# raguilar011095/planet_heightmap_generation

Measured on AMD Instinct MI355X. Metric: Mcells·iter/s, terrain-post erosion stack, higher is better.
Workload: dtype f64

## Files before the change

planet_heightmap_generation_amd/csrc/basin.hip:

```cpp
#include <hip/hip_runtime.h>

#include <string>

#include "device.h"

namespace wo {

namespace {

constexpr int32_t WO_RANGE_NONE = 0x7f7f7f7f;
#ifndef WO_BASIN_RANGE_SLOTS
#define WO_BASIN_RANGE_SLOTS 256
#endif
constexpr int WO_BASIN_RANGE = WO_BASIN_RANGE_SLOTS;
constexpr int WO_BASIN_KEY_BITS = 16;
constexpr int WO_BASIN_CHASE_CAP = 1 << 16;

__device__ inline int32_t basin_root(int32_t* J, int32_t s) {
    auto ld = [&](int32_t x) { return __atomic_load_n(&J[x], __ATOMIC_RELAXED); };
    int32_t j = ld(s), tort = j;
    int power = 1, lam = 0;
    for (int it = 0; it < WO_BASIN_CHASE_CAP; ++it) {
        const int32_t jj = ld(j);
        if (jj == j) return j;
        if (jj == tort) {
            int32_t m = jj, y = ld(jj);
            for (int k = 0; k < WO_BASIN_CHASE_CAP && y != jj; ++k) {
                const int32_t yy = ld(y);
                if (yy == y) return y;
                m = y < m ? y : m;
                y = yy;
            }
            __atomic_store_n(&J[m], m, __ATOMIC_RELAXED);
            return m;
// ... 72 lines not shown
    return __builtin_fma(r1, f1, r1);
}
__device__ inline double div_tail(double x, double y, double r) {
    const double q0 = x * r;
    const double e = __builtin_fma(-y, q0, x);
    return __builtin_fma(e, r, q0);
}
__device__ inline bool factor_ok(double f, float cellDistT, bool hasT2) {
    const bool fOk = f == 0.0 || (f >= 0x1p-300 && f <= 0x1p300);
    const bool dOk = !hasT2 || (cellDistT >= 0x1p-126f && cellDistT <= 0x1p100f);
    return fOk && dOk;
}
__device__ inline SolveOut solve_apply_recip(const SolveTask& T, double factor, double y1, double r1, double y2, double r2, double er, double et, double et2, int32_t tag) {
    const bool hasT = (T.flags & 4u) != 0, tOcean = (T.flags & 1u) != 0, hasT2 = (T.flags & 8u) != 0;
    const double hr = et > 0 ? et : 0;
    double hn = div_tail(er + factor * hr, y1, r1);
    hn = hn < hr ? hr : hn;
    hn = hn < 0 ? 0 : hn;
    const double eroded = er - hn;
    const double sl = div_tail(fabs(et - et2), y2, r2);
    const double slope = hasT2 ? sl : 0.0;
    const double depositFrac = 0.5 / (1 + slope * 50);
    const double deposit = eroded * depositFrac;
    float tv = (float)(et + deposit);
    tv = ((double)tv > hn) ? (float)hn : tv;
    const bool deposits = eroded > 0 && !tOcean;
    SolveOut o;
    o.self.tag = tag; o.dep.tag = tag;
    o.self.v = hasT ? (float)hn : (float)er;
    o.dep.v = hasT ? (deposits ? tv : (float)et) : 0.0f;
    return o;
}

template <int NW, bool STATS, int LAG_ = 2>
__global__ __launch_bounds__(64 * NW, (NW <= 4 ? 4 : 2)) void k_solve_flowing(Fields F, int32_t L, const int32_t* __restrict__ rangeStart, int32_t nRanges, int32_t launchTag,
                                                               int32_t* patchPending, int32_t* totalPending, const int32_t* __restrict__ big, const uint8_t* __restrict__ longFlag,
                                                               unsigned long long* stats) {
    constexpr int SC = 64 * NW;
    constexpr int LAG = LAG_, LOOKBACK = LAG + 2;
    constexpr int RCHUNKS = (LOOKBACK + LAG + 1 <= 8) ? 8 : 16;
    constexpr int RING = RCHUNKS * SC;
    static_assert(LOOKBACK + LAG + 1 <= RCHUNKS, "ring too small for the lag");
    __shared__ unsigned long long s_ring[2 * RING];
    __shared__ int32_t s_prog[NW];
    __shared__ int32_t s_level[STATS ? RING : 1];
    __shared__ int32_t s_maxLevel;
    __shared__ unsigned long long s_passes[STATS ? NW : 1], s_readyPasses[STATS ? NW : 1], s_clk[4];
    unsigned long long myPasses = 0, myReady = 0, cRead = 0, cTurn = 0, cRest = 0, cWait = 0;
    const int tid = threadIdx.x, wave = tid >> 6, lane = tid & 63;
    const long long cStart = STATS ? clock64() : 0;
    if (STATS && tid == 0) s_maxLevel = 0;
    int32_t S, E;
    if (!block_range(rangeStart, nRanges, L, big, longFlag, S, E)) return;
    const unsigned long long* G = reinterpret_cast<const unsigned long long*>(F.out);
    for (int i = tid; i < 2 * RING; i += SC) s_ring[i] = 0;
    if (tid < NW) s_prog[tid] = 0;
    __syncthreads();
    auto ring_put = [&](int32_t word, float v, int32_t tag) {
        __hip_atomic_store(&s_ring[word], (unsigned long long)__float_as_uint(v) | ((unsigned long long)(uint32_t)tag << 32), __ATOMIC_RELAXED, __HIP_MEMORY_SCOPE_WORKGROUP);
    };
    auto ring_get = [&](int32_t word) { return __hip_atomic_load(&s_ring[word], __ATOMIC_RELAXED, __HIP_MEMORY_SCOPE_WORKGROUP); };
    auto record = [&](int32_t q) { return F.task[q < L ? q : L - 1]; };
    auto far_index = [&](int32_t g, int32_t cbase) { const int32_t sq = g >> 1; return (g >= 0 && (sq < S || sq < cbase - LOOKBACK * SC)) ? g : 0; };
    SolveTask T1 = record(S + tid), T2 = record(S + SC + tid);
    unsigned long long a0 = G[far_index(T1.predSelf, S)], a1 = G[far_index(T1.predT, S)], a2 = G[far_index(T1.predT2, S)];
    SolveOut oPrev; oPrev.self.v = 0; oPrev.self.tag = 0; oPrev.dep.v = 0; oPrev.dep.tag = 0;
    bool storePrev = false;
    uint32_t fPrev = 0; int32_t rPrev = 0, tPrev = 0;
    auto store_prev = [&](int32_t slot) {
        F.out[slot] = oPrev;
        if (F.solveFinals) {
            if (fPrev & 16u) { F.e2[rPrev] = oPrev.self.v; F.me[rPrev] = oPrev.self.v; }
            if (fPrev & 32u) { F.e2[tPrev] = oPrev.dep.v; F.me[tPrev] = oPrev.dep.v; }
        }
    };
    int32_t ci = 0;
    for (int32_t base = S; base < E; base += SC, ++ci) {
        const int32_t q = base + tid;
        const bool mine = q < E;
        const long long cw0 = STATS ? clock64() : 0;
        if (ci > LAG) {
// ... 6 lines not shown
            }
            __builtin_amdgcn_fence(__ATOMIC_ACQUIRE, "workgroup");
        }
        const long long cw1 = STATS ? clock64() : 0;
        if (storePrev) store_prev(q - SC);
        const SolveTask T = T1;
        T1 = T2;
        T2 = record(base + 2 * SC + tid);
        const unsigned long long n0 = G[far_index(T1.predSelf, base + SC)], n1 = G[far_index(T1.predT, base + SC)], n2 = G[far_index(T1.predT2, base + SC)];
        double er = T.e0r, et = T.e0t, et2 = T.e0t2;
        bool blocked = false;
        const int32_t myWord = (2 * q) & (2 * RING - 1);
        int32_t r0 = -1, r1 = -1, r2 = -1, x0 = 0, x1 = 0, x2 = 0;
        if (mine) {
            auto classify = [&](int32_t g, unsigned long long far, double& v, int32_t& rw, int32_t& expect) {
                if (g < 0) return;
                const int32_t sq = g >> 1;
                if (sq >= q) { blocked = true; return; }
                if (sq >= S && sq >= base - LOOKBACK * SC) { rw = g & (2 * RING - 1); expect = sq + 1; return; }
                const int32_t tag = (int32_t)(far >> 32);
                const bool own = sq >= S;
                if (!own || tag != launchTag) { blocked = true; return; }
                v = __uint_as_float((uint32_t)far);
            };
            classify(T.predSelf, a0, er, r0, x0); classify(T.predT, a1, et, r1, x1); classify(T.predT2, a2, et2, r2, x2);
        }
        const int32_t w0 = r0 >= 0 ? r0 : myWord, w1 = r1 >= 0 ? r1 : myWord, w2 = r2 >= 0 ? r2 : myWord;
        const bool n0b = r0 >= 0, n1b = r1 >= 0, n2b = r2 >= 0;
        const float fr = (float)er, ft = (float)et, ft2 = (float)et2;
        const SolvePrepared pre = solve_prepare(T, F.solveK, F.solveM, F.solveDt);
        const double y1 = 1 + pre.factor, y2 = (double)T.cellDistT;
        const double rc1 = recip_refined(y1), rc2 = recip_refined(y2);
        const bool recipOk = !mine || factor_ok(pre.factor, T.cellDistT, (T.flags & 8u) != 0);
        bool open = mine;
        SolveOut o; o.self.v = 0; o.self.tag = 0; o.dep.v = 0; o.dep.tag = 0;
        if (mine && blocked) { ring_put(myWord, 0.0f, -(q + 1)); ring_put(myWord + 1, 0.0f, -(q + 1)); open = false; }
        const bool waveRecipOk = !__any(!recipOk);
        if (STATS) { const long long cw2 = clock64() + (long long)(__float_as_int((float)er) & 0); cRest += (unsigned long long)(cw2 - cw1); cWait += (unsigned long long)(cw1 - cw0); }
        while (__any(open)) {
            const long long c0 = STATS ? clock64() : 0;
            const unsigned long long g0 = ring_get(w0), g1 = ring_get(w1), g2 = ring_get(w2);
            const int32_t t0 = (int32_t)(g0 >> 32), t1 = (int32_t)(g1 >> 32), t2 = (int32_t)(g2 >> 32);
            const long long c1 = STATS ? (long long)(clock64() + (t0 & 0)) : 0;
            const bool ok = (!n0b | (t0 == x0)) & (!n1b | (t1 == x1)) & (!n2b | (t2 == x2));
            const bool bad = (n0b & (t0 == -x0)) | (n1b & (t1 == -x1)) | (n2b & (t2 == -x2));
            const bool ready = open & ok;
            if (STATS) { ++myPasses; if (__any(ready)) ++myReady; }
            if (__any(ready)) {
                const double ver = n0b ? (double)__uint_as_float((uint32_t)g0) : (double)fr;
                const double vet = n1b ? (double)__uint_as_float((uint32_t)g1) : (double)ft;
                const double vet2 = n2b ? (double)__uint_as_float((uint32_t)g2) : (double)ft2;
                const SolveOut oo = waveRecipOk ? solve_apply_recip(T, pre.factor, y1, rc1, y2, rc2, ver, vet, vet2, launchTag) : solve_apply_flat(T, pre, ver, vet, vet2, launchTag);
                if (ready) {
                    o = oo;
                    if (STATS && LAG_ != 3) {
                        int32_t lv = 0;
                        if (n0b) lv = max(lv, s_level[w0 >> 1]);
                        if (n1b) lv = max(lv, s_level[w1 >> 1]);
                        if (n2b) lv = max(lv, s_level[w2 >> 1]);
                        s_level[myWord >> 1] = lv + 1;
                        atomicMax(&s_maxLevel, lv + 1);
                    }
                    ring_put(myWord, oo.self.v, q + 1); ring_put(myWord + 1, oo.dep.v, q + 1);
                    open = false;
                }
            }
            const long long c2 = STATS ? clock64() : 0;
            if (STATS) { cRead += (unsigned long long)(c1 - c0); cTurn += (unsigned long long)(c2 - c1); }
            if (__any(open & bad)) {
                if (open & bad) { blocked = true; ring_put(myWord, 0.0f, -(q + 1)); ring_put(myWord + 1, 0.0f, -(q + 1)); open = false; }
            }
        }
        oPrev = o; storePrev = mine && !blocked; fPrev = T.flags; rPrev = T.pad_[0]; tPrev = T.pad_[1];
        if (mine && blocked) { atomicAdd(&patchPending[q / WO_PATCH], 1); atomicAdd(totalPending, 1); }
        a0 = n0; a1 = n1; a2 = n2;
        if (lane == 0) __hip_atomic_store(&s_prog[wave], ci + 1, __ATOMIC_RELEASE, __HIP_MEMORY_SCOPE_WORKGROUP);
    }
    if (storePrev) store_prev(S + ((E - S - 1) / SC) * SC + tid);
    if (STATS) {
        if (lane == 0) { s_passes[wave] = myPasses; s_readyPasses[wave] = myReady; }
        if (tid == 0) { s_clk[0] = cWait; s_clk[1] = cTurn; s_clk[2] = myPasses; s_clk[3] = cRest; }
        __syncthreads();
        if (tid == 0) {
            const unsigned long long c = (unsigned long long)(clock64() - cStart);
            const unsigned long long packed = (c << 24) | (unsigned long long)(s_maxLevel & 0xffffff);
            const unsigned long long old = atomicMax(&stats[0], packed);
            if (packed > old) {
                stats[1] = (unsigned long long)(E - S);
                unsigned long long mp = 0, mr = 0;
                for (int w = 0; w < NW; ++w) { mp = s_passes[w] > mp ? s_passes[w] : mp; mr = s_readyPasses[w] > mr ? s_readyPasses[w] : mr; }
                stats[2] = mp; stats[3] = mr; stats[4] = s_clk[0]; stats[5] = s_clk[1]; stats[6] = s_clk[2]; stats[7] = s_clk[3];
            }
        }
    }
}

}

void basin_alloc(wo_planet* p) {
    const int32_t N = p->N;
    hipStream_t s = cur_stream(p);
    if (!p->d_basinJ) {
        WO_HIP(hipMalloc((void**)&p->d_basinJ, (size_t)N * 4));
        WO_HIP(hipMalloc((void**)&p->d_basinSlot, (size_t)N * 4));
        WO_HIP(hipMalloc((void**)&p->d_basinKey, (size_t)N * 4));
        WO_HIP(hipMalloc((void**)&p->d_basinVals[0], (size_t)N * 4)); WO_HIP(hipMalloc((void**)&p->d_basinVals[1], (size_t)N * 4));
        WO_HIP(hipMalloc((void**)&p->d_basinRange, ((size_t)N / 64 + 8 + WO_LONG_MAX) * 4));
        WO_HIP(hipMalloc((void**)&p->d_basinLong, (size_t)N / 64 + 8));
        WO_HIP(hipMemsetAsync(p->d_basinSlot, 0xff, (size_t)N * 4, s));
    }
}

void basin_layout(wo_planet* p, bool slotIdentity) {
    const int32_t L = p->L;
    basin_alloc(p);
    int bitsL = 1;
    while (((int64_t)1 << bitsL) < (int64_t)L) ++bitsL;
    const int shift = bitsL > WO_BASIN_KEY_BITS ? bitsL - WO_BASIN_KEY_BITS : 0;
    const int grid = blocks_for(L, 1 << 16);
    launch(p, FAM_BASIN, k_basin_jump, grid, WO_BLOCK, slotIdentity ? (const int32_t*)nullptr : (const int32_t*)p->d_patchOrder, p->d_basinJ, L, (int32_t)shift, p->d_basinKey);
    const int rangeT = WO_BASIN_RANGE;
    const int nRanges = (int)(((int64_t)L + rangeT - 1) / rangeT);
    launch(p, FAM_BASIN, k_basin_keys, grid, WO_BLOCK, (const int32_t*)p->d_land[p->landCur], (const uint32_t*)p->d_basinKey, L, p->d_keys[0], p->d_basinVals[0],
           (int32_t)(p->opt.basinScramble ? 1 : 0), p->d_basinRange, (int32_t)(nRanges + 1));
    uint32_t* const kb[2] = {p->d_keys[0], p->d_keys[1]};
    int32_t* const vb[2] = {p->d_basinVals[0], p->d_basinVals[1]};
    const int sorted = radix_sort_pairs(p, FAM_BASIN_SORT, kb, vb, L, 0, 16 , p->d_basinSlot, radix_scratch(p, 1), p->N, p->rsFlip[1]);
    launch(p, FAM_BASIN, k_basin_slots, blocks_for(L, 4096), WO_BLOCK, (const int32_t*)p->d_basinVals[sorted], (const uint32_t*)p->d_keys[sorted], (int32_t*)nullptr, L, p->d_basinRange, (int32_t)rangeT);
    launch(p, FAM_BASIN, k_basin_long, blocks_for(nRanges), WO_BLOCK, (const int32_t*)p->d_basinRange, (int32_t)nRanges, L, p->d_basinRange + nRanges + 1, p->d_basinLong);
}

void basin_solve_launch(wo_planet* p, const Fields& F, int32_t launchTag, int32_t* totalPending) {
    const int nRanges = (int)(((int64_t)p->L + WO_BASIN_RANGE - 1) / WO_BASIN_RANGE);
    ++p->basinLaunches;
    const int32_t* big = (const int32_t*)(p->d_basinRange + nRanges + 1);
    const uint8_t* flag = (const uint8_t*)p->d_basinLong;
    const int grid = nRanges + WO_LONG_MAX;
    launch(p, FAM_SOLVE_BASIN, k_solve_flowing<2, false>, grid, 128, F, p->L, (const int32_t*)p->d_basinRange, (int32_t)nRanges, launchTag, p->d_patchPending, totalPending, big, flag, (unsigned long long*)nullptr);
}

void basin_free(wo_planet* p) {
    if (p->d_basinJ) (void)hipFree(p->d_basinJ);
    if (p->d_basinSlot) (void)hipFree(p->d_basinSlot);
    if (p->d_basinKey) (void)hipFree(p->d_basinKey);
    for (auto& v : p->d_basinVals) { if (v) (void)hipFree(v); v = nullptr; }
    if (p->d_basinRange) (void)hipFree(p->d_basinRange);
    if (p->d_basinLong) (void)hipFree(p->d_basinLong);
    p->d_basinLong = nullptr;
    p->d_basinJ = nullptr; p->d_basinSlot = nullptr; p->d_basinKey = nullptr; p->d_basinRange = nullptr;
}

}
```

planet_heightmap_generation_amd/csrc/device.h:

```cpp
#pragma once
#include <hip/hip_runtime.h>

#include <cstdint>
#include <cstdio>
#include <map>
#include <string>
#include <vector>

#include "host_util.h"

#include "erode_ops.h"
#include "flood_ops.h"
#include "wo_internal.h"

namespace wo {

struct HipError { std::string msg; };

#define WO_HIP(call)                                                                                   \
    do {                                                                                               \
        hipError_t e_ = (call);                                                                        \
        if (e_ != hipSuccess)                                                                          \
            throw ::wo::HipError{std::string(#call) + " -> " + hipGetErrorString(e_) + " (" + __FILE__ + ":" + \
                                 std::to_string(__LINE__) + ")"};                                      \
// ... 29 lines not shown
extern const char* const kFamilyNames[FAM_COUNT];

}

struct wo_ctx {
    int device = 0;
    hipStream_t stream = nullptr;
    hipDeviceProp_t prop{};
};

struct wo_flood_gpu {
    int64_t version = -1; int32_t L = 0, cap = 0, nSeeds = 0;
    int32_t *off = nullptr, *adj = nullptr, *cell = nullptr, *seedIdx = nullptr, *seeds = nullptr; double* nz = nullptr;
    float* e = nullptr;
    wo::FlHead *A = nullptr, *P = nullptr, *F = nullptr;
    unsigned long long *Astk = nullptr, *Pstk = nullptr, *Fstk = nullptr;
    int32_t *fdEpoch = nullptr, *inDirty = nullptr; uint8_t* isPending = nullptr;
    int32_t* lists[5] = {nullptr, nullptr, nullptr, nullptr, nullptr};
    void* ctrl = nullptr; void* h_ctrl = nullptr;
    int32_t *jump = nullptr, *outPar = nullptr, *outRoot = nullptr; float* outSurf = nullptr;
    int32_t *h_par = nullptr, *h_root = nullptr; float* h_surf = nullptr;
};

namespace wo {
struct Options {
    bool layoutIndex = false;
    bool tileLds = false;
    bool floodDevice = false;
    bool floodTiming = false;
    bool stageTimingAll = false;
    int  relaxedSortEvery = 1;
    bool relaxedFull = false;
    bool basinScramble = false;
    long long carveBudgetMs = 200;
    int  carveBlocks = 0;
    static Options from_env();
};
}

struct wo_planet {
    wo_ctx* ctx = nullptr;
    wo::Options opt;
    int32_t N = 0, E = 0, maxDeg = 0;
    wo::hvec<int32_t> h_off, h_adj;
    wo::hvec<float> h_xyz;
    wo::hvec<uint8_t> h_ocean;
    bool h_ocean_valid = false;
    float* h_pinned = nullptr;
    int32_t* h_count = nullptr;
    float* d_redoE = nullptr; int32_t* d_pendingEver = nullptr; int64_t redoCalls = 0;
    unsigned long long *h_word = nullptr, *d_word = nullptr; uint32_t wordSerial = 0;
    wo::FloodScratch flood;
    wo::FloodExchange floodX;
    void* floodLink = nullptr; void (*floodLinkFree)(void*) = nullptr;
    wo_flood_gpu fgpu;

    int32_t *d_off = nullptr, *d_adj = nullptr;
    float *d_dist = nullptr, *d_xyz = nullptr;
    float *d_e = nullptr, *d_e2 = nullptr, *d_hot = nullptr, *d_orig = nullptr;
    uint8_t *d_ocean = nullptr, *d_coast = nullptr;
    int64_t mirrorMaskVersion = -1;
    uint8_t* d_oceanKnown = nullptr; int32_t* d_maskDiff = nullptr; bool oceanKnownValid = false;
    bool hot_valid = false;
    float* d_savedE = nullptr; uint8_t* d_savedOcean = nullptr; bool saved = false;
    uint8_t* d_tables = nullptr;
    bool scratch = false;
    bool landIdentity = false;
    int64_t floodPrefixMirror = -1, floodPrefixStatic = -1;
    bool floodPrefixOk = false;
    int32_t *d_landIdx = nullptr, *d_land[2] = {nullptr, nullptr}, *d_rank = nullptr;
    int32_t* d_landInit = nullptr; int64_t oceanVersion = 0, landListsOcean = -1; bool landListsMirror = false; int32_t landListsL = -1;
    uint32_t* d_keys[2] = {nullptr, nullptr};
    float *d_cellDist = nullptr, *d_flow = nullptr;
    wo::SolveTask* d_task = nullptr; wo::SolveOut* d_out = nullptr; int32_t *d_haloSend = nullptr, *d_haloRecv = nullptr; float *d_haloBuf = nullptr, *h_haloBuf = nullptr; int32_t nHaloSend = 0, nHaloRecv = 0;
    int32_t* d_flowCnt = nullptr; wo::TargetRank* d_tr = nullptr; wo::EventList* d_ev = nullptr; float* d_me = nullptr;
    int32_t *d_carveSlot = nullptr, *d_carveDeps = nullptr, *d_carveDepCnt = nullptr, *d_carveDepPos = nullptr; uint32_t* d_rs[2] = {nullptr, nullptr}; int rsFlip[2] = {0, 0};    wo::CarveRec* d_carveRecs = nullptr; wo::CarveExpect* d_carveExpect = nullptr; unsigned long long* d_carveG = nullptr;    int32_t* d_carveSlotDone = nullptr; int64_t carveCap = 0;
    unsigned long long* d_accCnt = nullptr;
    int32_t *d_ftLr = nullptr, *d_ftParent = nullptr, *d_ftExtCnt = nullptr; uint32_t* d_ftInflow = nullptr; unsigned long long* d_ftRootAcc = nullptr;
    int32_t *d_jump = nullptr, *d_nj = nullptr;
    int32_t* d_doneAt = nullptr;
    double* d_totalExcess = nullptr;
    float *d_glac = nullptr, *d_iceFlow = nullptr;
    int32_t *d_iceTarget = nullptr, *d_arank = nullptr;
    uint8_t* d_iceUp = nullptr;
    int32_t *d_patchOrder = nullptr, *d_slotOf = nullptr, *d_patchPending = nullptr, *d_patchTotals = nullptr, *d_patchBlk = nullptr; int64_t patchVersion = -1; bool patchMirror = false; int32_t numPatches = 0; int64_t lastPatchLaunches = 1; int64_t solveCalls = 0;
    hipStream_t side = nullptr; hipEvent_t evFork = nullptr, evJoin = nullptr; bool onSide = false;
    uint32_t* d_basinKey = nullptr; int32_t* d_basinVals[2] = {nullptr, nullptr}; int32_t *d_basinJ = nullptr, *d_basinSlot = nullptr, *d_basinRange = nullptr; uint8_t* d_basinLong = nullptr; int64_t basinLaunches = 0; wo::Affine* d_affine[2] = {nullptr, nullptr};    int64_t solvePassSerial = 0;
    int32_t* h_patchTotals = nullptr;
    int32_t *d_listA = nullptr, *d_listB = nullptr, *d_counters = nullptr;
    void* d_sortTemp = nullptr; size_t sortTempBytes = 0;
    int landCur = 0;
    int32_t L = 0;

    struct Import {
        uint8_t* img = nullptr; int64_t imgCap = 0;
        int32_t* label = nullptr;
        uint8_t* flags = nullptr;
        int32_t* lists = nullptr;
        uint8_t* seedOcean = nullptr;
        int32_t* blockCounts = nullptr;
        int32_t* totals = nullptr; int32_t* h_totals = nullptr;
    } imp;

    struct wo_wind_block* wind = nullptr;

    struct Mirror {
        bool built = false, active = false;
        int32_t *perm = nullptr, *inv = nullptr, *off = nullptr, *adj = nullptr;
        float *dist = nullptr, *xyz = nullptr, *e = nullptr, *e2 = nullptr, *hot = nullptr;
        uint8_t *ocean = nullptr, *coast = nullptr;
        wo::hvec<int32_t> h_perm, h_morton;
        wo::hvec<uint8_t> h_mask;
        int64_t version = 0;
        int32_t *o_off = nullptr, *o_adj = nullptr; float *o_dist = nullptr, *o_xyz = nullptr, *o_e = nullptr, *o_e2 = nullptr;
        uint8_t *o_ocean = nullptr, *o_coast = nullptr;
    } mirror;

    hipEvent_t evStart = nullptr, evStop = nullptr;
    bool profiling = false;
// ... 67 lines not shown
```

planet_heightmap_generation_amd/csrc/erode_ops.h:

```cpp
#pragma once
#include <cmath>
#include <cstdint>
#include <cstring>

#include "noise.h"

namespace wo {

constexpr int WO_MAX_DEG = 24;
constexpr int32_t WO_NOT_DONE = 0x7fffffff;

#ifndef WO_TASK_ALIGN
#define WO_TASK_ALIGN 16
#endif
struct alignas(WO_TASK_ALIGN) SolveTask {
    int32_t predSelf, predT, predT2;
    uint32_t flags;
    float e0r, e0t, e0t2;
    float cellDistT;
    double factor;
    int32_t pad_[2];
};
static_assert(sizeof(SolveTask) == 48, "one 48-byte record per task");
#ifndef WO_PATCH_CELLS
// ... 503 lines not shown
    const double eroded = er - hn;
    float tval = (float)et;
    if (eroded > 0 && !(T.flags & 1u)) {
        double slope = 0;
        if (T.flags & 8u) slope = fabs(et - et2) / S.cellDistT;
        const double depositFrac = 0.5 / (1 + slope * 50);
        const double deposit = eroded * depositFrac;
        tval = (float)(et + deposit);
        if ((double)tval > hn) tval = (float)hn;
    }
    o.self.v = (float)hn; o.dep.v = tval;
    return o;
}
WO_HD inline SolveOut solve_apply_flat(const SolveTask& T, const SolvePrepared& S, double er, double et, double et2, int32_t tag) {
    const bool hasT = (T.flags & 4u) != 0, tOcean = (T.flags & 1u) != 0, hasT2 = (T.flags & 8u) != 0;
    const double hr = et > 0 ? et : 0;
    double hn = (er + S.factor * hr) / S.onePlusFactor;
    hn = hn < hr ? hr : hn;
    hn = hn < 0 ? 0 : hn;
    const double eroded = er - hn;
    const double sl = fabs(et - et2) / S.cellDistT;
    const double slope = hasT2 ? sl : 0.0;
    const double depositFrac = 0.5 / (1 + slope * 50);
    const double deposit = eroded * depositFrac;
    float tv = (float)(et + deposit);
    tv = ((double)tv > hn) ? (float)hn : tv;
    const bool deposits = eroded > 0 && !tOcean;
    SolveOut o;
    o.self.tag = tag; o.dep.tag = tag;
    o.self.v = hasT ? (float)hn : (float)er;
    o.dep.v = hasT ? (deposits ? tv : (float)et) : 0.0f;
    return o;
}
WO_HD inline SolveOut solve_compute(const SolveTask& T, double er, double et, double et2, int32_t tag, double K, double m, double dt) {
    return solve_apply(T, solve_prepare(T, K, m, dt), er, et, et2, tag);
}

WO_HD inline bool solve_task(const Fields& F, int32_t r, int32_t round, double K, double m, double dt) {
    const SolveTask T = F.task[r];
    const Granule* G = reinterpret_cast<const Granule*>(F.out);
    double er = T.e0r, et = T.e0t, et2 = T.e0t2;
    if (T.predSelf >= 0) { const Granule g = G[T.predSelf]; if (g.tag == 0 || !(g.tag < round)) return false; er = g.v; }
    if (T.predT >= 0)    { const Granule g = G[T.predT];    if (g.tag == 0 || !(g.tag < round)) return false; et = g.v; }
    if (T.predT2 >= 0)   { const Granule g = G[T.predT2];   if (g.tag == 0 || !(g.tag < round)) return false; et2 = g.v; }
    F.out[r] = solve_compute(T, er, et, et2, round, K, m, dt);
    return true;
}

WO_HD inline int32_t latest_event_cell(const Fields& F, int32_t x) {
    int32_t best = -1, bestRank = 0x7fffffff;
    { const TargetRank v = F.tr[x]; if (v.target >= 0) { best = x; bestRank = v.rank; } }
    int32_t b, nbs[WO_ROW];
    const int deg = load_row(F, x, b, nbs);
    if (deg <= WO_ROW) {
        TargetRank q[WO_ROW];
#pragma unroll
        for (int k = 0; k < WO_ROW; ++k) q[k] = F.tr[nbs[k]];
#pragma unroll
        for (int k = 0; k < WO_ROW; ++k) if (k < deg && q[k].target == x && q[k].rank < bestRank) { best = nbs[k]; bestRank = q[k].rank; }
    } else {
        for (int32_t j = b; j < b + deg; ++j) {
            const int32_t n = F.adj[j];
            const TargetRank v = F.tr[n];
            if (v.target != x) continue;
            if (v.rank < bestRank) { best = n; bestRank = v.rank; }
        }
// ... 453 lines not shown
```

planet_heightmap_generation_amd/csrc/planet.hip:

```cpp
#include <hip/hip_runtime.h>

#include <algorithm>
#include <atomic>
#include <chrono>
#include <cmath>
#include <cstring>

#include "../../include/worogen.h"
#include "device.h"
#include "elevation_host.h"
#include "elevation_kernels.h"
#include "kernels_impl.h"
#include "flood_kernels.h"
#include "elevation_bfs.h"
#include "noise.h"

namespace wo {

const char* const kFamilyNames[FAM_COUNT] = {
    "coast_flags", "smooth_elevation", "sharpen_ridges", "soil_creep", "warp_terrain", "noise_eval", "synthetic_terrain",
    "ocean_from_elevation", "sort_keys", "sort_radix", "rank_scatter", "receivers", "flow_climb",
    "flow_final", "solve_setup", "solve_round", "solve_final", "thermal_excess", "thermal_apply",
    "glac_index", "ice_receivers", "ice_round", "carve_setup", "carve_round", "moraine_fjord", "glacial_blend", "solve_patch", "elev_collisions", "elev_uplift_fused", "plate_grid", "plate_project", "smooth_field", "flood_eval", "flood_apply", "flood_misc", "climate_sweeps", "basin_layout", "basin_sort", "solve_basin", "flow_tiles", "misc", "event_pair_empty", "event_pair_noop_kernel", "event_pair_two_noop_kernels"};

// ... 458 lines not shown
        const int32_t N = p->N;
        launch(p, FAM_MISC, k_mirror_gather_f32, blocks_for(N, 4096), WO_BLOCK, (const float*)p->d_e, (const int32_t*)M.perm, M.e, N);
        launch(p, FAM_MISC, k_mirror_gather_u8, blocks_for(N, 4096), WO_BLOCK, (const uint8_t*)p->d_ocean, (const int32_t*)M.perm, M.ocean, N);
        M.o_off = p->d_off; M.o_adj = p->d_adj; M.o_dist = p->d_dist; M.o_xyz = p->d_xyz; M.o_e = p->d_e; M.o_e2 = p->d_e2; M.o_ocean = p->d_ocean; M.o_coast = p->d_coast;
        point_at_mirror(M.e, M.e2);
        M.active = on = true;
    }
    void suspend() {
        if (!on) return;
        auto& M = p->mirror;
        launch(p, FAM_MISC, k_mirror_scatter_f32, blocks_for(p->N, 4096), WO_BLOCK, (const float*)p->d_e, (const int32_t*)M.perm, M.o_e, p->N);
        cur = p->d_e; cur2 = p->d_e2;
        point_at_planet();
    }
    void resume() {
        if (!on) return;
        auto& M = p->mirror;
        launch(p, FAM_MISC, k_mirror_gather_f32, blocks_for(p->N, 4096), WO_BLOCK, (const float*)M.o_e, (const int32_t*)M.perm, cur, p->N);
        point_at_mirror(cur, cur2);
    }
    void finish() {
        if (!on) return;
        suspend();
        p->mirror.active = on = false;
    }
    ~MirrorScope() { if (on) { point_at_planet(); p->mirror.active = false; } }
};

static void ensure_side_stream(wo_planet* p) {
    if (p->side) return;
    int prLeast = 0, prGreatest = 0;
    WO_HIP(hipDeviceGetStreamPriorityRange(&prLeast, &prGreatest));
    WO_HIP(hipStreamCreateWithPriority(&p->side, hipStreamNonBlocking, prGreatest));
    WO_HIP(hipEventCreateWithFlags(&p->evFork, hipEventDisableTiming)); WO_HIP(hipEventCreateWithFlags(&p->evJoin, hipEventDisableTiming));
}

struct RedoWithChecks {};

struct ErodeCall {
    wo_planet* p;
    int32_t hIters; double K, m, dt; int32_t tIters; double talus, kThermal; int32_t gIters; double gStrength; bool checkEveryPass;
    int32_t total, midIter; double gCarve, gConv, gDep, gFjord;
    int gridN, gridL = 0;
    StageClock clk; MirrorScope mir; FloodRun floodRun;
    int64_t sorts = 0, maxSolve = 0, patchLaunches = 0, basinPasses = 0, basinLeftoverPasses = 0, iceRounds = 0, carveRounds = 0, carveActive = 0, carveFlowLeft = 0;
    double floodHostMs = 0;
    ErodeCall(wo_planet* pl, int32_t h, double K_, double m_, double dt_, int32_t t, double talus_, double kT, int32_t g, double gs, bool check)
        : p(pl), hIters(h), K(K_), m(m_), dt(dt_), tIters(t), talus(talus_), kThermal(kT), gIters(std::max(g, 0)), gStrength(gs != gs ? 0 : gs),
          checkEveryPass(check), total(std::max(hIters, std::max(tIters, gIters))), midIter((int32_t)std::floor(total * 0.75 + 0.5)),
          gridN(xcd_grid(pl->N)), clk(pl), mir(pl) {
        const double gScale = gIters > 0 ? 1.0 / gIters : 0;
        gCarve = 0.02 * gScale; gConv = 0.01 * gScale; gDep = 0.005 * gScale; gFjord = 0.015 * gScale;
    }
    void stats(bool mirrored) const {
        p->erodeStats = {{"land_cells", (double)p->L}, {"mirror_layout", mirrored ? 1.0 : 0.0}, {"iterations", (double)total}, {"sorts", (double)sorts},
                         {"solve_launches_max_per_pass", (double)maxSolve}, {"solve_patch_launches_total", (double)patchLaunches},
                         {"solve_basin_passes", (double)basinPasses}, {"solve_basin_passes_with_leftovers", (double)basinLeftoverPasses},
                         {"flow_two_level", (p->d_ftLr && p->landIdentity && hIters > 0) ? 1.0 : 0.0}, {"ice_rounds_total", (double)iceRounds},
                         {"carve_rounds_total", (double)carveRounds}, {"carve_active_total", (double)carveActive}, {"carve_flow_launches_with_leftovers", (double)carveFlowLeft}, {"solve_check_every_pass", checkEveryPass ? 1.0 : 0.0}, {"calls_run_again_with_checks", (double)p->redoCalls}, {"flood_stage_ms", floodHostMs},
                         {"flood_device_pass1_ms", floodRun.deviceMs}, {"flood_device_rounds", (double)floodRun.rounds}, {"flood_device_epochs", (double)floodRun.epochs},
                         {"flood_device_evaluations", (double)floodRun.evals}, {"flood_equal_key_decisions", (double)floodRun.ties}, {"flood_pass1_on_host", (floodRun.usedDevice && !floodRun.fellBack) ? 0.0 : 1.0},
                         {"flood_host_calls", (double)floodRun.host.calls}, {"flood_host_serial_pass1", (double)floodRun.host.serialPass1}, {"flood_host_tie_groups", (double)floodRun.host.tieGroups}, {"flood_host_contested", (double)floodRun.host.contested},
                         {"flood_host_open_parents", (double)floodRun.host.openParents}, {"flood_host_unresolved", (double)floodRun.host.unresolved},
                         {"flood_host_path_redo", (double)floodRun.host.pathRedo}, {"flood_host_replays", (double)floodRun.host.replays}, {"flood_host_replayed_landmasses", (double)floodRun.host.replayedLandmasses}, {"flood_host_pass1_ms", floodRun.host.pass1Ms},
                         {"flood_host_pass23_ms", floodRun.host.pass23Ms},
                         {"relaxed_sort_every", (double)p->opt.relaxedSortEvery}, {"relaxed_full", p->opt.relaxedFull ? 1.0 : 0.0}, {"flood_exchange_calls", (double)p->floodX.calls}, {"flood_exchange_gathers", (double)p->floodX.gathers}, {"flood_exchange_whole_planet_floods", (double)p->floodX.globalFloods}, {"flood_exchange_received", (double)p->floodX.received}};
    }
// ... 194 lines not shown
    if (!basin) return;
    ensure_side_stream(p);
    if (tilesBeforeFork) {
        launch(p, FAM_FLOW_TILES, k_flow_tiles<false>, flow_tile_count(p->L), FT_THREADS, F, FT);
        launch(p, FAM_FLOW_TILES, k_flow_root_links, blocks_for(p->L, 4096), WO_BLOCK, F, FT);
    }
    WO_HIP(hipEventRecord(p->evFork, s));
    WO_HIP(hipStreamWaitEvent(p->side, p->evFork, 0));
    p->onSide = true;
    try { basin_layout(p, slotIdentity); } catch (...) { p->onSide = false; throw; }
    p->onSide = false;
    WO_HIP(hipEventRecord(p->evJoin, p->side));
}
static void erode_flow(ErodeCall& c, const Fields& F, const FlowTiles& FT, int32_t* donorCnt, bool flowTiles, bool tilesBeforeFork, bool clearOut) {
    wo_planet* p = c.p;
    c.clk.begin("flow");
    if (flowTiles) {
        const int tiles = flow_tile_count(p->L);
        if (!tilesBeforeFork) {
            launch(p, FAM_FLOW_TILES, k_flow_tiles<false>, tiles, FT_THREADS, F, FT);
            launch(p, FAM_FLOW_TILES, k_flow_root_links, blocks_for(p->L, 4096), WO_BLOCK, F, FT);
        }
        launch(p, FAM_FLOW_TILES, k_flow_root_climb, blocks_for(p->L, 4096), WO_BLOCK, F, FT);
        launch(p, FAM_FLOW_TILES, k_flow_tiles<true>, tiles, FT_THREADS, F, FT);
    } else
        launch(p, FAM_FLOW_SNAP, k_flow_climb, c.gridL, WO_BLOCK, F, (const int32_t*)p->d_flowCnt, (int32_t)0x7fffffff);
    Fields Ff = F;
    if (p->opt.relaxedFull) Ff.ev = nullptr;
    launch(p, FAM_FLOW_FINAL, k_flow_final, c.gridL, WO_BLOCK, Ff, donorCnt, clearOut ? p->d_out : (SolveOut*)nullptr);
    c.clk.end();
}
static void erode_solve_basin(ErodeCall& c, Fields F, int32_t iter) {
    wo_planet* p = c.p; hipStream_t s = p->ctx->stream;
    WO_HIP(hipStreamWaitEvent(s, p->evJoin, 0));
    F.slotOf = p->d_basinSlot; F.solveLean = 1;
    const bool unchecked = !c.checkEveryPass; F.solveFinals = unchecked ? 1 : 0;
    launch(p, FAM_SOLVE_SETUP, k_solve_setup_batched<true>, c.gridL, WO_BLOCK, F, p->d_patchPending, (int32_t)p->numPatches, p->d_patchTotals, (int32_t)WO_PATCH_TOTAL_SLOTS);
    int32_t passTag = 1;
    if (unchecked) {
        if (p->solvePassSerial >= 0x3ff00000) { WO_HIP(hipMemsetAsync(p->d_out, 0, (size_t)p->N * sizeof(SolveOut), s)); p->solvePassSerial = 0; }
        passTag = (1 << 20) + (int32_t)(++p->solvePassSerial);
    }
    const int64_t r = run_solve_patches(p, F, c.K, c.m, c.dt, unchecked, passTag);
    ++c.basinPasses; if (r > 1) ++c.basinLeftoverPasses;
    c.patchLaunches += r; c.maxSolve = std::max(c.maxSolve, r);
    if (!unchecked) launch(p, FAM_SOLVE_FINAL, k_solve_final, c.gridL, WO_BLOCK, F, p->d_e2, (iter < c.tIters) ? p->d_me : (float*)nullptr);
}
static void erode_solve_affine(ErodeCall& c, const Fields& F) {
    wo_planet* p = c.p;
    if (!p->d_affine[0]) { p->d_affine[0] = dalloc<Affine>((size_t)p->N); p->d_affine[1] = dalloc<Affine>((size_t)p->N); }
    launch(p, FAM_SOLVE_SETUP, k_affine_init, c.gridL, WO_BLOCK, F, p->d_affine[0]);
    int cur = 0;
    for (int q = 0; q < 12; ++q, cur ^= 1) launch(p, FAM_SOLVE_ROUND, k_affine_jump, c.gridL, WO_BLOCK, F, (const Affine*)p->d_affine[cur], p->d_affine[cur ^ 1]);
    launch(p, FAM_SOLVE_FINAL, k_affine_apply, c.gridL, WO_BLOCK, F, (const Affine*)p->d_affine[cur], p->d_e2);
}
static void hydraulic_step(ErodeCall& c, int32_t iter) {
    wo_planet* p = c.p;
    Fields F = p->fields();
    F.solveK = c.K; F.solveM = c.m; F.solveDt = c.dt;
    const bool basin = !p->opt.relaxedFull;
    const bool slotIdentity = c.mir.on && p->mirror.h_mask.size() == (size_t)p->N;
    if (basin) { basin_alloc(p); F.basinMslot = slotIdentity ? nullptr : p->d_slotOf; }
    const bool flowTiles = p->landIdentity;
    FlowTiles FT = flowTiles ? flow_tiles_buffers(p) : FlowTiles{};
    const bool tilesBeforeFork = basin && flowTiles && slotIdentity;
    if (tilesBeforeFork) FT.basinJ = p->d_basinJ;
    int32_t* const donorCnt = flowTiles ? (int32_t*)nullptr : p->d_flowCnt;
    erode_receivers(c, F, FT, donorCnt, basin, slotIdentity, tilesBeforeFork);
    erode_flow(c, F, FT, donorCnt, flowTiles, tilesBeforeFork, basin && c.checkEveryPass);
    c.clk.begin("solve");
    if (basin) erode_solve_basin(c, F, iter); else erode_solve_affine(c, F);
    swap_elev(p);
    c.clk.end();
}
static void thermal_step(ErodeCall& c, bool afterSolve) {
// ... 107 lines not shown
    ~DevBufs() { for (void* b : bufs) (void)hipFree(b); }
    template <class T> T* up(const T* host, size_t n, hipStream_t s) {
        if (!host) return nullptr;
        void* d = nullptr; WO_HIP(hipMalloc(&d, std::max<size_t>(n, 1) * sizeof(T))); bufs.push_back(d);
        WO_HIP(hipMemcpyAsync(d, host, n * sizeof(T), hipMemcpyHostToDevice, s));
        return (T*)d;
    }
    template <class T> T* alloc(size_t n) { void* d = nullptr; WO_HIP(hipMalloc(&d, std::max<size_t>(n, 1) * sizeof(T))); bufs.push_back(d); return (T*)d; }
};
ClimateMesh climate_mesh(const wo_planet* p) { ClimateMesh M; M.N = p->N; M.off = p->d_off; M.adj = p->d_adj; M.xyz = p->d_xyz; return M; }
}


using namespace wo;

#define WO_TRY try {
#define WO_CATCH(fn)                                                                   \
    } catch (const HipError& e) { set_error(std::string(fn) + ": " + e.msg); return 2; } \
      catch (const std::exception& e) { set_error(std::string(fn) + ": " + e.what()); return 3; }

Options Options::from_env() {
    auto str = [](const char* n) { const char* v = std::getenv(n); return std::string(v ? v : ""); };
    auto on = [](const char* n) { const char* v = std::getenv(n); return v && std::atoi(v) != 0; };
    auto set = [](const char* n) { return std::getenv(n) != nullptr; };
    Options o;
    o.layoutIndex = str("WO_LAYOUT") == "index";
    o.tileLds = on("WO_TILE_LDS");
    o.floodDevice = str("WO_FLOOD") == "device";
    o.floodTiming = set("WO_FLOOD_TIMING");
    o.stageTimingAll = str("WO_STAGE_TIMING") == "all";
    if (set("WO_RELAXED_SORT_EVERY")) o.relaxedSortEvery = std::max(1, std::atoi(std::getenv("WO_RELAXED_SORT_EVERY")));
    o.relaxedFull = str("WO_RELAXED") == "full";
    o.basinScramble = test_hook_int("basin_scramble", 0) != 0;
    o.carveBudgetMs = test_hook_int("carve_budget_ms", 200);
    o.carveBlocks = (int)std::max<long long>(0, test_hook_int("carve_blocks", 0));
    return o;
}

float* wo::smooth_field_resident(wo_planet* p, float* a, float* b, int32_t passes) {
    Fields F = p->fields();
    for (int32_t pass = 0; pass < passes; ++pass) {
        launch(p, FAM_SMOOTH_FIELD, k_smooth_field, xcd_grid(p->N), WO_BLOCK, F, (const float*)a, b);
        std::swap(a, b);
    }
    return a;
}

bool wo::check_planet(wo_planet* p, const char* fn) {
    if (!p) { set_error(std::string(fn) + ": null planet handle"); return false; }
    p->opt = Options::from_env();
    hipError_t e = hipSetDevice(p->ctx->device);
    if (e != hipSuccess) { set_error(std::string(fn) + ": hipSetDevice failed: " + hipGetErrorString(e)); return false; }
    return true;
}

static void erode_composite_checked(wo_planet* p, int32_t hIters, double K, double m, double dt, int32_t tIters, double talus,
                                    double kThermal, int32_t gIters, double gStrength) {
    if (hIters <= 0 || p->floodX.on) { erode_composite(p, hIters, K, m, dt, tIters, talus, kThermal, gIters, gStrength, true); return; }
    hipStream_t s = p->ctx->stream;
    if (!p->d_redoE) p->d_redoE = dalloc<float>((size_t)p->N);
    if (!p->d_pendingEver) p->d_pendingEver = dalloc<int32_t>(16);
    WO_HIP(hipMemcpyAsync(p->d_redoE, p->d_e, (size_t)p->N * sizeof(float), hipMemcpyDeviceToDevice, s));
    WO_HIP(hipMemsetAsync(p->d_pendingEver, 0, 16 * sizeof(int32_t), s));
    try {
        erode_composite(p, hIters, K, m, dt, tIters, talus, kThermal, gIters, gStrength, false);
    } catch (const RedoWithChecks&) {
// ... 82 lines not shown
        if (neighborDist) {
            WO_HIP(hipMemcpyAsync(p->d_dist, neighborDist, (size_t)E * 4, hipMemcpyHostToDevice, s));
        } else {
            std::vector<float> nd(E);
            neighbor_dist(N, adjOffset, adjList, r_xyz, nd.data());
            WO_HIP(hipMemcpyAsync(p->d_dist, nd.data(), (size_t)E * 4, hipMemcpyHostToDevice, s));
            WO_HIP(hipStreamSynchronize(s));
        }
        WO_HIP(hipMemsetAsync(p->d_e, 0, (size_t)N * 4, s));
        WO_HIP(hipMemsetAsync(p->d_ocean, 0, (size_t)N, s));
        WO_HIP(hipEventCreate(&p->evStart)); WO_HIP(hipEventCreate(&p->evStop));
        WO_HIP(hipStreamSynchronize(s));
        return p;
    } catch (const HipError& e) {
        set_error(std::string("wo_planet_create: ") + e.msg);
        if (p) wo_planet_destroy(p);
        return nullptr;
    }
}

void wo_planet_destroy(wo_planet* p) {
    if (!p) return;
    (void)hipSetDevice(p->ctx->device);
    (void)hipStreamSynchronize(p->ctx->stream);
    dfree(p->d_off); dfree(p->d_adj); dfree(p->d_dist); dfree(p->d_xyz); dfree(p->d_e); dfree(p->d_e2); dfree(p->d_hot); dfree(p->d_orig);
    flood_gpu_free(p->fgpu);
    if (p->floodLink && p->floodLinkFree) p->floodLinkFree(p->floodLink);
    p->floodLink = nullptr;
    basin_free(p);
    import_free(p);
    wind_free(p);
    if (p->side) { (void)hipStreamSynchronize(p->side); (void)hipStreamDestroy(p->side); p->side = nullptr; }
    if (p->evFork) { (void)hipEventDestroy(p->evFork); p->evFork = nullptr; }
    if (p->evJoin) { (void)hipEventDestroy(p->evJoin); p->evJoin = nullptr; }
    mirror_free(p);
    dfree(p->d_ocean); dfree(p->d_coast); dfree(p->d_tables); dfree(p->d_savedE); dfree(p->d_savedOcean);
    if (p->d_oceanKnown) { (void)hipFree(p->d_oceanKnown); p->d_oceanKnown = nullptr; } if (p->d_maskDiff) { (void)hipFree(p->d_maskDiff); p->d_maskDiff = nullptr; }
    dfree(p->d_landInit); dfree(p->d_landIdx); dfree(p->d_land[0]); dfree(p->d_land[1]); dfree(p->d_keys[0]); dfree(p->d_keys[1]); dfree(p->d_rank);
    dfree(p->d_cellDist); dfree(p->d_flow); dfree(p->d_task); dfree(p->d_out); dfree(p->d_flowCnt); dfree(p->d_tr); dfree(p->d_ev); dfree(p->d_me); dfree(p->d_haloSend); dfree(p->d_haloRecv); dfree(p->d_haloBuf); if (p->h_haloBuf) { (void)hipHostFree(p->h_haloBuf); p->h_haloBuf = nullptr; } dfree(p->d_carveSlot); dfree(p->d_redoE); dfree(p->d_pendingEver); for (auto& r : p->d_rs) { if (r) (void)hipFree(r); r = nullptr; } dfree(p->d_carveG); dfree(p->d_carveExpect); dfree(p->d_carveRecs); dfree(p->d_carveSlotDone); dfree(p->d_carveDeps); dfree(p->d_carveDepCnt); dfree(p->d_carveDepPos); dfree(p->d_ftLr); dfree(p->d_ftParent); dfree(p->d_affine[0]); dfree(p->d_affine[1]); dfree(p->d_ftExtCnt); dfree(p->d_ftInflow); dfree(p->d_ftRootAcc); dfree(p->d_accCnt); dfree(p->d_jump); dfree(p->d_nj);
    dfree(p->d_doneAt); dfree(p->d_totalExcess);
    dfree(p->d_glac); dfree(p->d_iceFlow); dfree(p->d_iceTarget); dfree(p->d_arank); dfree(p->d_iceUp);
    dfree(p->d_patchOrder); dfree(p->d_slotOf); dfree(p->d_patchPending); dfree(p->d_patchTotals); dfree(p->d_patchBlk);
    dfree(p->d_listA); dfree(p->d_listB); dfree(p->d_counters);
    if (p->h_patchTotals) (void)hipHostFree(p->h_patchTotals);
    if (p->d_sortTemp) (void)hipFree(p->d_sortTemp);
    if (p->h_pinned) (void)hipHostFree(p->h_pinned);
    if (p->h_count) (void)hipHostFree(p->h_count);
    if (p->h_word) { (void)hipHostFree(p->h_word); p->h_word = nullptr; }
    for (auto& pe : p->pending) { (void)hipEventDestroy(pe.a); (void)hipEventDestroy(pe.b); }
    for (auto& b : p->stageBrackets) { (void)hipEventDestroy(b.a); (void)hipEventDestroy(b.b); }
    for (auto e : p->eventPool) (void)hipEventDestroy(e);
    if (p->evStart) (void)hipEventDestroy(p->evStart);
    if (p->evStop) (void)hipEventDestroy(p->evStop);
    delete p;
}

int wo_planet_upload(wo_planet* p, const float* r_elevation, const uint8_t* r_isOcean) {
    if (!check_planet(p, "wo_planet_upload")) return 1;
    WO_TRY
    hipStream_t s = p->ctx->stream;
    if (r_elevation) WO_HIP(hipMemcpyAsync(p->d_e, r_elevation, (size_t)p->N * 4, hipMemcpyHostToDevice, s));
    if (r_isOcean) {
        WO_HIP(hipMemcpyAsync(p->d_ocean, r_isOcean, (size_t)p->N, hipMemcpyHostToDevice, s));
        if (p->h_ocean.size() != (size_t)p->N || std::memcmp(p->h_ocean.data(), r_isOcean, (size_t)p->N) != 0) {
            p->h_ocean.assign(r_isOcean, r_isOcean + p->N);
            p->flood.staticValid = false; ++p->oceanVersion;
// ... 677 lines not shown
```

Baseline: 6272.

## Split basin solve into height and deferred deposit phases; wait on slots event earlier

The flowing solve kernel now computes and publishes only the height value on the critical dependency chain. The deposit value, which needs a second division, is computed later during passes where no lane in the wave was ready, so idle spin passes absorb that work. Separately, the main stream now waits on a new event recorded right after the basin sort, and only waits for the full join before the patch solve, so setup overlaps the slot and long-range kernels. This adds an extra loop state and more branching, and the deposit write can lag behind readers that need it.

```diff
diff --git a/planet_heightmap_generation_amd/csrc/basin.hip b/planet_heightmap_generation_amd/csrc/basin.hip
--- a/planet_heightmap_generation_amd/csrc/basin.hip
+++ b/planet_heightmap_generation_amd/csrc/basin.hip
@@ -1,5 +1,7 @@
 #include <hip/hip_runtime.h>
 
+#include <cstdio>
+#include <cstdlib>
 #include <string>
 
 #include "device.h"
@@ -138,10 +140,12 @@
     return o;
 }
 
+struct SolveDivRecip { double y, r; __device__ double operator()(double x) const { return div_tail(x, y, r); } };
+
 template <int NW, bool STATS, int LAG_ = 2>
 __global__ __launch_bounds__(64 * NW, (NW <= 4 ? 4 : 2)) void k_solve_flowing(Fields F, int32_t L, const int32_t* __restrict__ rangeStart, int32_t nRanges, int32_t launchTag,
                                                                int32_t* patchPending, int32_t* totalPending, const int32_t* __restrict__ big, const uint8_t* __restrict__ longFlag,
-                                                               unsigned long long* stats) {
+                                                               int32_t depositEveryPass, unsigned long long* stats) {
     constexpr int SC = 64 * NW;
     constexpr int LAG = LAG_, LOOKBACK = LAG + 2;
     constexpr int RCHUNKS = (LOOKBACK + LAG + 1 <= 8) ? 8 : 16;
@@ -151,8 +155,8 @@
     __shared__ int32_t s_prog[NW];
     __shared__ int32_t s_level[STATS ? RING : 1];
     __shared__ int32_t s_maxLevel;
-    __shared__ unsigned long long s_passes[STATS ? NW : 1], s_readyPasses[STATS ? NW : 1], s_clk[4];
-    unsigned long long myPasses = 0, myReady = 0, cRead = 0, cTurn = 0, cRest = 0, cWait = 0;
+    __shared__ unsigned long long s_passes[STATS ? NW : 1], s_readyPasses[STATS ? NW : 1], s_depositPasses[STATS ? NW : 1], s_clk[6];
+    unsigned long long myPasses = 0, myReady = 0, myDeposit = 0, cRead = 0, cTurn = 0, cDeposit = 0, cRest = 0, cWait = 0;
     const int tid = threadIdx.x, wave = tid >> 6, lane = tid & 63;
     const long long cStart = STATS ? clock64() : 0;
     if (STATS && tid == 0) s_maxLevel = 0;
@@ -225,12 +229,15 @@
         const double y1 = 1 + pre.factor, y2 = (double)T.cellDistT;
         const double rc1 = recip_refined(y1), rc2 = recip_refined(y2);
         const bool recipOk = !mine || factor_ok(pre.factor, T.cellDistT, (T.flags & 8u) != 0);
-        bool open = mine;
+        bool open = mine, owes = false;
         SolveOut o; o.self.v = 0; o.self.tag = 0; o.dep.v = 0; o.dep.tag = 0;
         if (mine && blocked) { ring_put(myWord, 0.0f, -(q + 1)); ring_put(myWord + 1, 0.0f, -(q + 1)); open = false; }
         const bool waveRecipOk = !__any(!recipOk);
+        const SolveDivRecip byY1{y1, rc1}, byY2{y2, rc2};
+        const SolveDivBy flatY1{pre.onePlusFactor}, flatY2{pre.cellDistT};
+        double hEt = 0, hEt2 = 0, hHn = 0, hEroded = 0; bool hDeposits = false;
         if (STATS) { const long long cw2 = clock64() + (long long)(__float_as_int((float)er) & 0); cRest += (unsigned long long)(cw2 - cw1); cWait += (unsigned long long)(cw1 - cw0); }
-        while (__any(open)) {
+        while (__any(open | owes)) {
             const long long c0 = STATS ? clock64() : 0;
             const unsigned long long g0 = ring_get(w0), g1 = ring_get(w1), g2 = ring_get(w2);
             const int32_t t0 = (int32_t)(g0 >> 32), t1 = (int32_t)(g1 >> 32), t2 = (int32_t)(g2 >> 32);
@@ -238,14 +245,16 @@
             const bool ok = (!n0b | (t0 == x0)) & (!n1b | (t1 == x1)) & (!n2b | (t2 == x2));
             const bool bad = (n0b & (t0 == -x0)) | (n1b & (t1 == -x1)) | (n2b & (t2 == -x2));
             const bool ready = open & ok;
-            if (STATS) { ++myPasses; if (__any(ready)) ++myReady; }
-            if (__any(ready)) {
+            const bool anyReady = __any(ready);
+            if (STATS) { ++myPasses; if (anyReady) ++myReady; }
+            if (anyReady) {
                 const double ver = n0b ? (double)__uint_as_float((uint32_t)g0) : (double)fr;
                 const double vet = n1b ? (double)__uint_as_float((uint32_t)g1) : (double)ft;
                 const double vet2 = n2b ? (double)__uint_as_float((uint32_t)g2) : (double)ft2;
-                const SolveOut oo = waveRecipOk ? solve_apply_recip(T, pre.factor, y1, rc1, y2, rc2, ver, vet, vet2, launchTag) : solve_apply_flat(T, pre, ver, vet, vet2, launchTag);
+                const SolveHeight H = waveRecipOk ? solve_height_phase(T.flags, pre.factor, byY1, ver, vet) : solve_height_phase(T.flags, pre.factor, flatY1, ver, vet);
                 if (ready) {
-                    o = oo;
+                    o.self.v = H.selfV; o.self.tag = launchTag;
+                    hEt = vet; hEt2 = vet2; hHn = H.hn; hEroded = H.eroded; hDeposits = H.deposits;
                     if (STATS && LAG_ != 3) {
                         int32_t lv = 0;
                         if (n0b) lv = max(lv, s_level[w0 >> 1]);
@@ -254,12 +263,22 @@
                         s_level[myWord >> 1] = lv + 1;
                         atomicMax(&s_maxLevel, lv + 1);
                     }
-                    ring_put(myWord, oo.self.v, q + 1); ring_put(myWord + 1, oo.dep.v, q + 1);
-                    open = false;
+                    ring_put(myWord, H.selfV, q + 1);
+                    open = false; owes = true;
                 }
             }
             const long long c2 = STATS ? clock64() : 0;
-            if (STATS) { cRead += (unsigned long long)(c1 - c0); cTurn += (unsigned long long)(c2 - c1); }
+            if ((!anyReady | (depositEveryPass != 0)) && __any(owes)) {
+                if (STATS) ++myDeposit;
+                const float dv = waveRecipOk ? solve_deposit_phase(T.flags, byY2, hEt, hEt2, hHn, hEroded, hDeposits) : solve_deposit_phase(T.flags, flatY2, hEt, hEt2, hHn, hEroded, hDeposits);
+                if (owes) {
+                    o.dep.v = dv; o.dep.tag = launchTag;
+                    ring_put(myWord + 1, dv, q + 1);
+                    owes = false;
+                }
+            }
+            const long long c3 = STATS ? clock64() : 0;
+            if (STATS) { cRead += (unsigned long long)(c1 - c0); cTurn += (unsigned long long)(c2 - c1); cDeposit += (unsigned long long)(c3 - c2); }
             if (__any(open & bad)) {
                 if (open & bad) { blocked = true; ring_put(myWord, 0.0f, -(q + 1)); ring_put(myWord + 1, 0.0f, -(q + 1)); open = false; }
             }
@@ -271,8 +290,8 @@
     }
     if (storePrev) store_prev(S + ((E - S - 1) / SC) * SC + tid);
     if (STATS) {
-        if (lane == 0) { s_passes[wave] = myPasses; s_readyPasses[wave] = myReady; }
-        if (tid == 0) { s_clk[0] = cWait; s_clk[1] = cTurn; s_clk[2] = myPasses; s_clk[3] = cRest; }
+        if (lane == 0) { s_passes[wave] = myPasses; s_readyPasses[wave] = myReady; s_depositPasses[wave] = myDeposit; }
+        if (tid == 0) { s_clk[0] = cWait; s_clk[1] = cTurn; s_clk[2] = myPasses; s_clk[3] = cRest; s_clk[4] = cDeposit; s_clk[5] = cRead; }
         __syncthreads();
         if (tid == 0) {
             const unsigned long long c = (unsigned long long)(clock64() - cStart);
@@ -280,9 +299,10 @@
             const unsigned long long old = atomicMax(&stats[0], packed);
             if (packed > old) {
                 stats[1] = (unsigned long long)(E - S);
-                unsigned long long mp = 0, mr = 0;
-                for (int w = 0; w < NW; ++w) { mp = s_passes[w] > mp ? s_passes[w] : mp; mr = s_readyPasses[w] > mr ? s_readyPasses[w] : mr; }
+                unsigned long long mp = 0, mr = 0, md = 0;
+                for (int w = 0; w < NW; ++w) { mp = s_passes[w] > mp ? s_passes[w] : mp; mr = s_readyPasses[w] > mr ? s_readyPasses[w] : mr; md = s_depositPasses[w] > md ? s_depositPasses[w] : md; }
                 stats[2] = mp; stats[3] = mr; stats[4] = s_clk[0]; stats[5] = s_clk[1]; stats[6] = s_clk[2]; stats[7] = s_clk[3];
+                stats[8] = md; stats[9] = s_clk[4]; stats[10] = s_clk[5];
             }
         }
     }
@@ -319,6 +339,7 @@
     uint32_t* const kb[2] = {p->d_keys[0], p->d_keys[1]};
     int32_t* const vb[2] = {p->d_basinVals[0], p->d_basinVals[1]};
     const int sorted = radix_sort_pairs(p, FAM_BASIN_SORT, kb, vb, L, 0, 16 , p->d_basinSlot, radix_scratch(p, 1), p->N, p->rsFlip[1]);
+    WO_HIP(hipEventRecord(p->evSlots, cur_stream(p)));
     launch(p, FAM_BASIN, k_basin_slots, blocks_for(L, 4096), WO_BLOCK, (const int32_t*)p->d_basinVals[sorted], (const uint32_t*)p->d_keys[sorted], (int32_t*)nullptr, L, p->d_basinRange, (int32_t)rangeT);
     launch(p, FAM_BASIN, k_basin_long, blocks_for(nRanges), WO_BLOCK, (const int32_t*)p->d_basinRange, (int32_t)nRanges, L, p->d_basinRange + nRanges + 1, p->d_basinLong);
 }
@@ -329,7 +350,20 @@
     const int32_t* big = (const int32_t*)(p->d_basinRange + nRanges + 1);
     const uint8_t* flag = (const uint8_t*)p->d_basinLong;
     const int grid = nRanges + WO_LONG_MAX;
-    launch(p, FAM_SOLVE_BASIN, k_solve_flowing<2, false>, grid, 128, F, p->L, (const int32_t*)p->d_basinRange, (int32_t)nRanges, launchTag, p->d_patchPending, totalPending, big, flag, (unsigned long long*)nullptr);
+#ifdef WO_BASIN_STATS_BUILD
+    const char* at = std::getenv("WO_BASIN_STATS");
+    if (at && p->basinLaunches == std::atoll(at)) {
+        hipStream_t s = cur_stream(p);
+        unsigned long long* d = nullptr; unsigned long long h[16] = {0};
+        WO_HIP(hipMalloc((void**)&d, sizeof h)); WO_HIP(hipMemsetAsync(d, 0, sizeof h, s));
+        launch(p, FAM_SOLVE_BASIN, k_solve_flowing<2, true>, grid, 128, F, p->L, (const int32_t*)p->d_basinRange, (int32_t)nRanges, launchTag, p->d_patchPending, totalPending, big, flag, (int32_t)(p->opt.solveDepositEveryPass ? 1 : 0), d);
+        WO_HIP(hipMemcpyAsync(h, d, sizeof h, hipMemcpyDeviceToHost, s)); WO_HIP(hipStreamSynchronize(s)); (void)hipFree(d);
+        std::fprintf(stderr, "basin stats: launch %lld slowest range: clocks %llu slots %llu depth %llu | passes %llu height %llu deposit %llu | wave 0 clocks: wait %llu read %llu height %llu deposit %llu rest %llu\n",
+                     (long long)p->basinLaunches, h[0] >> 24, h[1], h[0] & 0xffffffull, h[2], h[3], h[8], h[4], h[10], h[5], h[9], h[7]);
+        return;
+    }
+#endif
+    launch(p, FAM_SOLVE_BASIN, k_solve_flowing<2, false>, grid, 128, F, p->L, (const int32_t*)p->d_basinRange, (int32_t)nRanges, launchTag, p->d_patchPending, totalPending, big, flag, (int32_t)(p->opt.solveDepositEveryPass ? 1 : 0), (unsigned long long*)nullptr);
 }
 
 void basin_free(wo_planet* p) {
diff --git a/planet_heightmap_generation_amd/csrc/device.h b/planet_heightmap_generation_amd/csrc/device.h
--- a/planet_heightmap_generation_amd/csrc/device.h
+++ b/planet_heightmap_generation_amd/csrc/device.h
@@ -85,6 +85,7 @@
     int  relaxedSortEvery = 1;
     bool relaxedFull = false;
     bool basinScramble = false;
+    bool solveDepositEveryPass = false;
     long long carveBudgetMs = 200;
     int  carveBlocks = 0;
     static Options from_env();
@@ -137,7 +138,7 @@
     int32_t *d_iceTarget = nullptr, *d_arank = nullptr;
     uint8_t* d_iceUp = nullptr;
     int32_t *d_patchOrder = nullptr, *d_slotOf = nullptr, *d_patchPending = nullptr, *d_patchTotals = nullptr, *d_patchBlk = nullptr; int64_t patchVersion = -1; bool patchMirror = false; int32_t numPatches = 0; int64_t lastPatchLaunches = 1; int64_t solveCalls = 0;
-    hipStream_t side = nullptr; hipEvent_t evFork = nullptr, evJoin = nullptr; bool onSide = false;
+    hipStream_t side = nullptr; hipEvent_t evFork = nullptr, evSlots = nullptr, evJoin = nullptr; bool onSide = false;
     uint32_t* d_basinKey = nullptr; int32_t* d_basinVals[2] = {nullptr, nullptr}; int32_t *d_basinJ = nullptr, *d_basinSlot = nullptr, *d_basinRange = nullptr; uint8_t* d_basinLong = nullptr; int64_t basinLaunches = 0; wo::Affine* d_affine[2] = {nullptr, nullptr};    int64_t solvePassSerial = 0;
     int32_t* h_patchTotals = nullptr;
     int32_t *d_listA = nullptr, *d_listB = nullptr, *d_counters = nullptr;
diff --git a/planet_heightmap_generation_amd/csrc/erode_ops.h b/planet_heightmap_generation_amd/csrc/erode_ops.h
--- a/planet_heightmap_generation_amd/csrc/erode_ops.h
+++ b/planet_heightmap_generation_amd/csrc/erode_ops.h
@@ -559,6 +559,33 @@
     o.dep.v = hasT ? (deposits ? tv : (float)et) : 0.0f;
     return o;
 }
+struct SolveDivBy { double y; WO_HD double operator()(double x) const { return x / y; } };
+struct SolveHeight { double hn, eroded; float selfV; bool deposits; };
+template <class Div>
+WO_HD inline SolveHeight solve_height_phase(uint32_t flags, double factor, const Div& byOnePlusFactor, double er, double et) {
+    const bool hasT = (flags & 4u) != 0, tOcean = (flags & 1u) != 0;
+    const double hr = et > 0 ? et : 0;
+    double hn = byOnePlusFactor(er + factor * hr);
+    hn = hn < hr ? hr : hn;
+    hn = hn < 0 ? 0 : hn;
+    SolveHeight H;
+    H.hn = hn;
+    H.eroded = er - hn;
+    H.deposits = H.eroded > 0 && !tOcean;
+    H.selfV = hasT ? (float)hn : (float)er;
+    return H;
+}
+template <class Div>
+WO_HD inline float solve_deposit_phase(uint32_t flags, const Div& byCellDistT, double et, double et2, double hn, double eroded, bool deposits) {
+    const bool hasT = (flags & 4u) != 0, hasT2 = (flags & 8u) != 0;
+    const double sl = byCellDistT(fabs(et - et2));
+    const double slope = hasT2 ? sl : 0.0;
+    const double depositFrac = 0.5 / (1 + slope * 50);
+    const double deposit = eroded * depositFrac;
+    float tv = (float)(et + deposit);
+    tv = ((double)tv > hn) ? (float)hn : tv;
+    return hasT ? (deposits ? tv : (float)et) : 0.0f;
+}
 WO_HD inline SolveOut solve_compute(const SolveTask& T, double er, double et, double et2, int32_t tag, double K, double m, double dt) {
     return solve_apply(T, solve_prepare(T, K, m, dt), er, et, et2, tag);
 }
diff --git a/planet_heightmap_generation_amd/csrc/planet.hip b/planet_heightmap_generation_amd/csrc/planet.hip
--- a/planet_heightmap_generation_amd/csrc/planet.hip
+++ b/planet_heightmap_generation_amd/csrc/planet.hip
@@ -514,7 +514,7 @@
     int prLeast = 0, prGreatest = 0;
     WO_HIP(hipDeviceGetStreamPriorityRange(&prLeast, &prGreatest));
     WO_HIP(hipStreamCreateWithPriority(&p->side, hipStreamNonBlocking, prGreatest));
-    WO_HIP(hipEventCreateWithFlags(&p->evFork, hipEventDisableTiming)); WO_HIP(hipEventCreateWithFlags(&p->evJoin, hipEventDisableTiming));
+    WO_HIP(hipEventCreateWithFlags(&p->evFork, hipEventDisableTiming)); WO_HIP(hipEventCreateWithFlags(&p->evSlots, hipEventDisableTiming)); WO_HIP(hipEventCreateWithFlags(&p->evJoin, hipEventDisableTiming));
 }
 
 struct RedoWithChecks {};
@@ -775,7 +775,7 @@
 }
 static void erode_solve_basin(ErodeCall& c, Fields F, int32_t iter) {
     wo_planet* p = c.p; hipStream_t s = p->ctx->stream;
-    WO_HIP(hipStreamWaitEvent(s, p->evJoin, 0));
+    WO_HIP(hipStreamWaitEvent(s, p->evSlots, 0));
     F.slotOf = p->d_basinSlot; F.solveLean = 1;
     const bool unchecked = !c.checkEveryPass; F.solveFinals = unchecked ? 1 : 0;
     launch(p, FAM_SOLVE_SETUP, k_solve_setup_batched<true>, c.gridL, WO_BLOCK, F, p->d_patchPending, (int32_t)p->numPatches, p->d_patchTotals, (int32_t)WO_PATCH_TOTAL_SLOTS);
@@ -784,6 +784,7 @@
         if (p->solvePassSerial >= 0x3ff00000) { WO_HIP(hipMemsetAsync(p->d_out, 0, (size_t)p->N * sizeof(SolveOut), s)); p->solvePassSerial = 0; }
         passTag = (1 << 20) + (int32_t)(++p->solvePassSerial);
     }
+    WO_HIP(hipStreamWaitEvent(s, p->evJoin, 0));
     const int64_t r = run_solve_patches(p, F, c.K, c.m, c.dt, unchecked, passTag);
     ++c.basinPasses; if (r > 1) ++c.basinLeftoverPasses;
     c.patchLaunches += r; c.maxSolve = std::max(c.maxSolve, r);
@@ -957,6 +958,7 @@
     if (set("WO_RELAXED_SORT_EVERY")) o.relaxedSortEvery = std::max(1, std::atoi(std::getenv("WO_RELAXED_SORT_EVERY")));
     o.relaxedFull = str("WO_RELAXED") == "full";
     o.basinScramble = test_hook_int("basin_scramble", 0) != 0;
+    o.solveDepositEveryPass = test_hook_int("solve_deposit_every_pass", 0) != 0;
     o.carveBudgetMs = test_hook_int("carve_budget_ms", 200);
     o.carveBlocks = (int)std::max<long long>(0, test_hook_int("carve_blocks", 0));
     return o;
@@ -1105,6 +1107,7 @@
     wind_free(p);
     if (p->side) { (void)hipStreamSynchronize(p->side); (void)hipStreamDestroy(p->side); p->side = nullptr; }
     if (p->evFork) { (void)hipEventDestroy(p->evFork); p->evFork = nullptr; }
+    if (p->evSlots) { (void)hipEventDestroy(p->evSlots); p->evSlots = nullptr; }
     if (p->evJoin) { (void)hipEventDestroy(p->evJoin); p->evJoin = nullptr; }
     mirror_free(p);
     dfree(p->d_ocean); dfree(p->d_coast); dfree(p->d_tables); dfree(p->d_savedE); dfree(p->d_savedOcean);
```

Result: slower. 5702 (-9.1%).
